# davidbau/rewriting

Measured on NVIDIA H100. Metric: StyleGAN2-256 images/sec, higher is better.
Workload: dtype bf16x3 (3-term split bf16 operands, fp32 accumulate; fp32 in/out)

## Files before the change

### rewriting_b200/csrc/conv_tc.cu

```cuda
#include <cstdlib>
#include <cstring>

#include "rw_common.cuh"
#include "rw_kernels.h"

namespace rw {

namespace {

constexpr int BM = 128;
constexpr int BK = 32;
constexpr int MMA_K = 16;
constexpr int kStages = 7;
constexpr int kNumThreads = 384;
constexpr int kTmaWarp = 8;
constexpr uint32_t kProducerRegs = 40;
constexpr uint32_t kConsumerRegs = 232;
constexpr int kCluster = 2;
constexpr int kChunkKB = 16;

template <int BN>
struct ConvSmem {
  static constexpr int kABytes = BM * BK * 2;
  static constexpr int kBBytes = BN * BK * 2;
  static constexpr int kStageBytes = 2 * kABytes + 2 * kBBytes;
  static constexpr int kTotal = kStages * kStageBytes + 512  + 256 ;
};
static_assert(ConvSmem<128>::kTotal <= 232448, "conv_tc: shared memory over the per-block limit");

struct Barriers {
  uint64_t full[kStages];
  uint64_t empty[kStages];
};

__device__ __forceinline__ void decode_tile(int tile, int nphase, int nsched, int& ph, int& mn) {
  mn = tile / nphase;
  ph = tile - mn * nphase;
  if (nphase > 1) ph = (ph + ((nsched % nphase) == 0 ? tile / nsched : mn)) % nphase;
}

template <int BN, int EPI, bool PROF>
__global__ void __launch_bounds__(kNumThreads, 1)
conv_tc_kernel(const __grid_constant__ CUtensorMap map_a_hi,
               const __grid_constant__ CUtensorMap map_a_lo,
               const __grid_constant__ CUtensorMap map_w_hi,
               const __grid_constant__ CUtensorMap map_w_lo, const ConvTcParams p) {
  extern __shared__ uint8_t smem_raw[];
  uint8_t* smem = reinterpret_cast<uint8_t*>((reinterpret_cast<uintptr_t>(smem_raw) + 511) &
                                             ~static_cast<uintptr_t>(511));
  using S = ConvSmem<BN>;
  constexpr int NR = BN / 2;
  constexpr int NJ = BN / 8;
  Barriers* bars = reinterpret_cast<Barriers*>(smem + kStages * S::kStageBytes);

  const int warp = __shfl_sync(0xffffffffu, static_cast<int>(threadIdx.x >> 5), 0);
  const int lane = threadIdx.x & 31;
  const int rank = static_cast<int>(cluster_ctarank());
  const int nsched = static_cast<int>(num_clusters_x());
  const int first_unit = static_cast<int>(cluster_id_x());

  const int m_tiles = (p.rows + BM - 1) / BM;
  const int n_tiles = p.Cout / BN;
  const int mn_units = (m_tiles + kCluster - 1) / kCluster * n_tiles;
  const int num_units = mn_units * p.nphase;
  const int kb_per_tap = p.Cin / BK;

  if (warp == kTmaWarp && lane == 0) {
    tma_prefetch_desc(&map_a_hi);
    tma_prefetch_desc(&map_a_lo);
    tma_prefetch_desc(&map_w_hi);
    tma_prefetch_desc(&map_w_lo);
    for (int s = 0; s < kStages; ++s) {
      mbar_init(&bars->full[s], 1);
      mbar_init(&bars->empty[s], 2 * kCluster);
    }
    fence_mbar_init();
  }
  cluster_sync();

  if (warp < kTmaWarp) {
    setmaxnreg_inc<kConsumerRegs>();
    const int wg = threadIdx.x >> 7;
    const int c = lane & 3;
    const int img = p.Hp * p.Wp;
    auto release = [&](int s) {
      if ((threadIdx.x & 127) == 0) {
#pragma unroll
        for (int r = 0; r < kCluster; ++r) mbar_arrive_cluster(mapa_shared(&bars->empty[s], r));
      }
    };
    auto clk = [] { return static_cast<uint32_t>(clock()); };
    uint32_t prof[6] = {0, 0, 0, 0, 0, 0};
    uint32_t tp0 = 0, tp1 = 0;
    if constexpr (PROF) prof[5] = 0u - clk();
    int stage = 0;
    uint32_t phase = 0;
    for (int unit = first_unit; unit < num_units; unit += nsched) {
      int ph, mn;
      decode_tile(unit, p.nphase, nsched, ph, mn);
      const int num_kb = p.ph_ntaps[ph] * kb_per_tap;
      const int n_tile = mn % n_tiles;
      const int n0 = n_tile * BN;
      const int m0 = ((mn / n_tiles) * kCluster + rank) * BM;

      float acc[NR], d[NR];
#pragma unroll
      for (int j = 0; j < NR; ++j) acc[j] = 0.f;
      for (int kb0 = 0; kb0 < num_kb; kb0 += kChunkKB) {
        const int kb_end = (kb0 + kChunkKB < num_kb) ? kb0 + kChunkKB : num_kb;
        int held = -1;
        for (int kb = kb0; kb < kb_end; ++kb) {
          if constexpr (PROF) tp0 = clk();
          mbar_wait(&bars->full[stage], phase);
          if constexpr (PROF) { tp1 = clk(); prof[0] += tp1 - tp0; }
          const uint32_t sa = smem_u32(smem + stage * S::kStageBytes);
          const uint64_t da_hi = make_smem_desc(sa + wg * (S::kABytes / 2), 16, 512, 2);
          const uint64_t da_lo = make_smem_desc(sa + S::kABytes + wg * (S::kABytes / 2), 16, 512, 2);
          const uint64_t db_hi = make_smem_desc(sa + 2 * S::kABytes, 16, 512, 2);
          const uint64_t db_lo = make_smem_desc(sa + 2 * S::kABytes + S::kBBytes, 16, 512, 2);
          wgmma_fence();
#pragma unroll
          for (int kk = 0; kk < BK / MMA_K; ++kk) {
            const uint64_t adv = static_cast<uint64_t>((kk * MMA_K * 2) >> 4);
            wgmma_m64nN<0, 0>(d, da_lo + adv, db_hi + adv, ((kb - kb0) | kk) != 0);
            wgmma_m64nN<0, 0>(d, da_hi + adv, db_lo + adv, 1u);
            wgmma_m64nN<0, 0>(d, da_hi + adv, db_hi + adv, 1u);
          }
          wgmma_commit();
          wgmma_wait<1>();
          if (held >= 0) release(held);
          held = stage;
          if (++stage == kStages) { stage = 0; phase ^= 1u; }
          if constexpr (PROF) prof[1] += clk() - tp1;
        }
        if constexpr (PROF) tp0 = clk();
        wgmma_wait<0>();
        release(held);
#pragma unroll
        for (int j = 0; j < NR; ++j) acc[j] += d[j];
        if constexpr (PROF) prof[2] += clk() - tp0;
      }
      if constexpr (PROF) tp0 = clk();

      uint32_t tid;
      asm volatile("mov.u32 %0, %%tid.x;\n" : "=r"(tid));
      const int row0 = m0 + ((tid >> 7) << 6) + (((tid >> 5) & 3) << 4) + ((tid & 31) >> 2);
#pragma unroll
      for (int i = 0; i < 2; ++i) {
        const int prow = row0 + 8 * i;
        const int b = prow / img;
        const int rem = prow - b * img;
        const int yy = rem / p.Wp;
        const int xx = rem - yy * p.Wp;
        const int Hv = p.ph_Hv[ph], Wv = p.ph_Wv[ph];
        const bool in_rows = prow < p.rows;
        const bool valid = in_rows && (yy < Hv) && (xx < Wv);
        const float* scl = (p.scale_bo && in_rows) ? p.scale_bo + static_cast<size_t>(b) * p.Cout : nullptr;
        float* outp = (p.out != nullptr && p.out_mode == 0 && valid)
                          ? p.out + p.ph_out_ofs[ph] + static_cast<size_t>(b) * p.out_sb +
                                static_cast<size_t>(yy) * p.out_sy + static_cast<size_t>(xx) * p.out_sx
                          : nullptr;
        if (EPI == 1 || !valid) {
          if (scl && (EPI == 1 || p.out_mode == 1)) {
#pragma unroll
            for (int j = 0; j < NJ; ++j) {
              const float2 sv = __ldg(reinterpret_cast<const float2*>(scl + n0 + 8 * j + 2 * c));
              acc[4 * j + 2 * i] *= sv.x;
              acc[4 * j + 2 * i + 1] *= sv.y;
            }
          }
          if (EPI == 1 && outp) {
#pragma unroll
            for (int j = 0; j < NJ; ++j)
#pragma unroll
              for (int e = 0; e < 2; ++e)
                outp[static_cast<size_t>(n0 + 8 * j + 2 * c + e) * p.out_sc] = acc[4 * j + 2 * i + e];
          }
        } else {
          float nz = 0.f;
          if (p.noise != nullptr)
            nz = __ldg(p.noise_w) * __ldg(p.noise + static_cast<size_t>(b) * p.noise_bstride +
                                          static_cast<size_t>(yy) * Wv + xx);
          const float act_gain = p.act_gain != 0.f ? p.act_gain : 1.4142135623730951f;
          if (scl) {
            const float* sc = scl + n0 + 2 * c;
#pragma unroll
            for (int j = 0; j < NJ; ++j)
#pragma unroll
              for (int e = 0; e < 2; ++e) acc[4 * j + 2 * i + e] *= __ldg(sc + 8 * j + e);
          }
#pragma unroll
          for (int j = 0; j < NJ; ++j)
#pragma unroll
            for (int e = 0; e < 2; ++e) acc[4 * j + 2 * i + e] += nz;
          if (p.bias) {
            const float* bi = p.bias + n0 + 2 * c;
#pragma unroll
            for (int j = 0; j < NJ; ++j)
#pragma unroll
              for (int e = 0; e < 2; ++e) acc[4 * j + 2 * i + e] += __ldg(bi + 8 * j + e);
          }
          if (p.act) {
#pragma unroll
            for (int j = 0; j < 2 * NJ; ++j) {
              float& t = acc[4 * (j >> 1) + 2 * i + (j & 1)];
              t = (t > 0.f ? t : 0.2f * t) * act_gain;
            }
          }
          if (outp) {
#pragma unroll
            for (int j = 0; j < NJ; ++j)
#pragma unroll
              for (int e = 0; e < 2; ++e)
                outp[static_cast<size_t>(n0 + 8 * j + 2 * c + e) * p.out_sc] = acc[4 * j + 2 * i + e];
          }
        }
        if (EPI == 0 && p.rgb_w != nullptr) {
          const float* rw0 = p.rgb_w + (static_cast<size_t>(valid ? b : 0) * 3) * p.Cout + n0 + 2 * c;
          const float* rw1 = rw0 + p.Cout;
          const float* rw2 = rw1 + p.Cout;
#pragma unroll
          for (int half = 0; half < BN / 64; ++half) {
            float r0 = 0.f, r1 = 0.f, r2 = 0.f;
            if (valid) {
#pragma unroll
              for (int j = 8 * half; j < 8 * half + 8; ++j)
#pragma unroll
                for (int e = 0; e < 2; ++e) {
                  const float t = acc[4 * j + 2 * i + e];
                  r0 = fmaf(__ldg(rw0 + 8 * j + e), t, r0);
                  r1 = fmaf(__ldg(rw1 + 8 * j + e), t, r1);
                  r2 = fmaf(__ldg(rw2 + 8 * j + e), t, r2);
                }
            }
#pragma unroll
            for (int s = 1; s < 4; s <<= 1) {
              r0 += __shfl_xor_sync(0xffffffffu, r0, s);
              r1 += __shfl_xor_sync(0xffffffffu, r1, s);
              r2 += __shfl_xor_sync(0xffffffffu, r2, s);
            }
            if (valid && c == 0) {
              const size_t hw = static_cast<size_t>(Hv) * Wv;
              float* rp = p.rgb_part + ((static_cast<size_t>(n_tile * (BN / 64) + half) * p.B + b) * 3) * hw +
                          static_cast<size_t>(yy) * Wv + xx;
              rp[0] = r0;
              rp[hw] = r1;
              rp[2 * hw] = r2;
            }
          }
        }
        if (p.out != nullptr && p.out_mode == 1 && in_rows) {
          float* orow = p.out + (static_cast<size_t>(ph) * p.rows + prow) * p.Cout + n0 + 2 * c;
#pragma unroll
          for (int j = 0; j < NJ; ++j)
            *reinterpret_cast<float2*>(orow + 8 * j) = make_float2(acc[4 * j + 2 * i], acc[4 * j + 2 * i + 1]);
        }
        if (EPI == 0 && p.next_hi != nullptr && in_rows) {
          const float* ns = p.next_scale + static_cast<size_t>(valid ? b : 0) * p.Cout + n0 + 2 * c;
          const size_t ofs = static_cast<size_t>(prow) * p.Cout + n0 + 2 * c;
          uint32_t* nh = reinterpret_cast<uint32_t*>(static_cast<__nv_bfloat16*>(p.next_hi) + ofs);
          uint32_t* nl = reinterpret_cast<uint32_t*>(static_cast<__nv_bfloat16*>(p.next_lo) + ofs);
#pragma unroll
          for (int j = 0; j < NJ; ++j) {
            float k0 = 0.f, k1 = 0.f;
            if (valid) {
              const float2 sv = __ldg(reinterpret_cast<const float2*>(ns + 8 * j));
              k0 = sv.x * acc[4 * j + 2 * i];
              k1 = sv.y * acc[4 * j + 2 * i + 1];
            }
            const __nv_bfloat162 hh = __floats2bfloat162_rn(k0, k1);
            const float2 hf = __bfloat1622float2(hh);
            const __nv_bfloat162 ll = __floats2bfloat162_rn(k0 - hf.x, k1 - hf.y);
            nh[4 * j] = *reinterpret_cast<const uint32_t*>(&hh);
            nl[4 * j] = *reinterpret_cast<const uint32_t*>(&ll);
          }
        }
      }
      if constexpr (PROF) { prof[3] += clk() - tp0; prof[4] += 1; }
    }
    if constexpr (PROF) {
      prof[5] += clk();
      if (lane == 0) {
        long long* dst = p.debug_prof + (static_cast<size_t>(blockIdx.x) * 8 + warp) * 8;
#pragma unroll
        for (int i = 0; i < 8; ++i) dst[i] = i < 6 ? prof[i] : 0;
      }
    }
  } else {
    setmaxnreg_dec<kProducerRegs>();
    if (warp == kTmaWarp && lane == 0) {
      constexpr uint16_t kMask = (1u << kCluster) - 1;
      constexpr int kBSlice = BN / kCluster;
      const uint32_t b_off = 2 * S::kABytes + rank * (S::kBBytes / kCluster);
      int stage = 0;
      uint32_t phase = 0;
      for (int unit = first_unit; unit < num_units; unit += nsched) {
        int ph, mn;
        decode_tile(unit, p.nphase, nsched, ph, mn);
        const int n0 = (mn % n_tiles) * BN + rank * kBSlice;
        const int m0 = ((mn / n_tiles) * kCluster + rank) * BM;
        for (int t = 0; t < p.ph_ntaps[ph]; ++t) {
          const int arow = m0 + p.ph_shift[ph][t];
          const int wcol = p.ph_kofs[ph][t];
          const int acol = p.ph_acol[ph][t];
          for (int kb = 0; kb < kb_per_tap; ++kb) {
            mbar_wait(&bars->empty[stage], phase ^ 1u);
            uint8_t* st = smem + stage * S::kStageBytes;
            mbar_expect_tx(&bars->full[stage], S::kStageBytes);
            tma_load_2d(st, &map_a_hi, &bars->full[stage], acol + kb * BK, arow);
            tma_load_2d(st + S::kABytes, &map_a_lo, &bars->full[stage], acol + kb * BK, arow);
            tma_load_2d_multicast(st + b_off, &map_w_hi, &bars->full[stage], wcol + kb * BK, n0,
                                  kMask);
            tma_load_2d_multicast(st + b_off + S::kBBytes, &map_w_lo, &bars->full[stage],
                                  wcol + kb * BK, n0, kMask);
            if (++stage == kStages) { stage = 0; phase ^= 1u; }
          }
        }
      }
    }
    __syncwarp();
  }
  cluster_sync();
}

}

template <int BN, int EPI, bool PROF>
static int conv_tc_launch_epi(const ConvTcParams& p, const void* a_hi, const void* a_lo,
                              const void* w_hi, const void* w_lo, int wk_total,
                              cudaStream_t stream) {
  CUtensorMap ma_hi, ma_lo, mw_hi, mw_lo;
  int rc;
  const uint64_t a_cols = p.a_cols > 0 ? p.a_cols : p.Cin;
  const uint64_t a_dims[2] = {a_cols, static_cast<uint64_t>(p.rows)}, a_str[1] = {a_cols * 2};
  const uint64_t w_dims[2] = {static_cast<uint64_t>(wk_total), static_cast<uint64_t>(p.Cout)};
  const uint64_t w_str[1] = {static_cast<uint64_t>(wk_total) * 2};
  const uint32_t a_box[2] = {BK, BM}, w_box[2] = {BK, BN / kCluster};
  if ((rc = make_tmap_nd_bf16(&ma_hi, a_hi, 2, a_dims, a_str, a_box, nullptr, 3))) return rc;
  if ((rc = make_tmap_nd_bf16(&ma_lo, a_lo, 2, a_dims, a_str, a_box, nullptr, 3))) return rc;
  if ((rc = make_tmap_nd_bf16(&mw_hi, w_hi, 2, w_dims, w_str, w_box, nullptr, 3))) return rc;
  if ((rc = make_tmap_nd_bf16(&mw_lo, w_lo, 2, w_dims, w_str, w_box, nullptr, 3))) return rc;

  cudaLaunchConfig_t cfg = {};
  cudaLaunchAttribute attr[1];
  attr[0].id = cudaLaunchAttributeClusterDimension;
  attr[0].val.clusterDim.x = kCluster;
  attr[0].val.clusterDim.y = 1;
  attr[0].val.clusterDim.z = 1;
  cfg.blockDim = dim3(kNumThreads);
  cfg.dynamicSmemBytes = ConvSmem<BN>::kTotal;
  cfg.stream = stream;
  cfg.attrs = attr;
  cfg.numAttrs = 1;
  static int max_clusters = 0;
  if (max_clusters == 0) {
    rc = check_cuda(cudaFuncSetAttribute(conv_tc_kernel<BN, EPI, PROF>,
                                         cudaFuncAttributeMaxDynamicSharedMemorySize, ConvSmem<BN>::kTotal),
                    "conv_tc smem attr");
    if (rc) return rc;
    cfg.gridDim = dim3(kCluster * (device_sm_count() / kCluster));
    rc = check_cuda(cudaOccupancyMaxActiveClusters(&max_clusters, conv_tc_kernel<BN, EPI, PROF>, &cfg),
                    "conv_tc cluster occupancy");
    if (rc) return rc;
    if (max_clusters < 1) {
      set_last_error("conv_tc: no cluster of %d CTAs fits on the device", kCluster);
      return RW_ERR_UNSUPPORTED;
    }
  }
  const int m_tiles = (p.rows + BM - 1) / BM;
  const int n_tiles = p.Cout / BN;
  const int num_units = (m_tiles + kCluster - 1) / kCluster * n_tiles * p.nphase;
  const int clusters = max_clusters < num_units ? max_clusters : num_units;
  cfg.gridDim = dim3(kCluster * clusters);
  rc = check_cuda(cudaLaunchKernelEx(&cfg, conv_tc_kernel<BN, EPI, PROF>, ma_hi, ma_lo, mw_hi, mw_lo, p),
                  "conv_tc launch");
  if (rc) return rc;
  return check_cuda(cudaGetLastError(), "conv_tc launch");
}

template <int BN>
static int conv_tc_launch_bn(const ConvTcParams& p, const void* a_hi, const void* a_lo,
                             const void* w_hi, const void* w_lo, int wk_total, cudaStream_t stream) {
  const bool lean = !p.noise && !p.bias && !p.act && !p.rgb_w && !p.rgb_part && !p.next_hi &&
                    p.out != nullptr && (reinterpret_cast<uintptr_t>(p.scale_bo) & 7u) == 0;
  if (p.debug_prof) return conv_tc_launch_epi<BN, 0, true>(p, a_hi, a_lo, w_hi, w_lo, wk_total, stream);
  if (lean) return conv_tc_launch_epi<BN, 1, false>(p, a_hi, a_lo, w_hi, w_lo, wk_total, stream);
  return conv_tc_launch_epi<BN, 0, false>(p, a_hi, a_lo, w_hi, w_lo, wk_total, stream);
}

int conv_tc_launch(const ConvTcParams& p, const void* a_hi, const void* a_lo, const void* w_hi,
                   const void* w_lo, int wk_total, cudaStream_t stream) {
  if (p.Cin % 64 != 0 || p.Cout % 64 != 0 || p.nphase < 1 || p.nphase > 4 || p.rows <= 0) {
    set_last_error("conv_tc: unsupported shape Cin=%d Cout=%d nphase=%d rows=%d", p.Cin, p.Cout,
                   p.nphase, p.rows);
    return RW_ERR_BAD_ARG;
  }
  for (int i = 0; i < p.nphase; ++i)
    if (p.ph_ntaps[i] < 1 || p.ph_ntaps[i] > 9) {
      set_last_error("conv_tc: phase %d has %d taps", i, p.ph_ntaps[i]);
      return RW_ERR_BAD_ARG;
    }
  const struct {
    const void* ptr;
    unsigned align;
    const char* name;
  } need[] = {
      {p.scale_bo, p.out_mode == 1 ? 8u : 4u, "scale_bo"},
      {p.out, p.out_mode == 1 ? 8u : 4u, "out"},
      {p.noise, 4u, "noise"},
      {p.noise_w, 4u, "noise_w"},
      {p.bias, 4u, "bias"},
      {p.next_scale, 8u, "next_scale"},
      {p.next_hi, 4u, "next_hi"},
      {p.next_lo, 4u, "next_lo"},
      {p.rgb_w, 4u, "rgb_w"},
      {p.rgb_part, 4u, "rgb_part"},
  };
  for (const auto& n : need)
    if (n.ptr != nullptr && (reinterpret_cast<uintptr_t>(n.ptr) & (n.align - 1)) != 0) {
      set_last_error("conv_tc: %s (%p) is not %u-byte aligned", n.name, n.ptr, n.align);
      return RW_ERR_BAD_ARG;
    }
  if (p.Cout % 128 == 0) return conv_tc_launch_bn<128>(p, a_hi, a_lo, w_hi, w_lo, wk_total, stream);
  return conv_tc_launch_bn<64>(p, a_hi, a_lo, w_hi, w_lo, wk_total, stream);
}

}
```

Measured before the change: 2046.

## Add dedicated epilogue warpgroup with shared-memory accumulator handoff

Splits the consumer into two MMA warpgroups plus a new epilogue warpgroup. MMA warps write their accumulators to a per-warpgroup shared-memory handoff buffer, signalled by acc_full/acc_empty mbarriers, so the epilogue (scaling, bf16 hi/lo split, stores) overlaps the next tile's main loop. In exchange the MMA warps get fewer registers, the block grows to 512 threads, and the BN=128 pipeline drops from 7 to 5 stages to make room for the handoff buffers, which may expose more TMA latency.

After: 2072, median of 6. 1.01x the previous value.

```diff
diff --git a/rewriting_b200/csrc/conv_tc.cu b/rewriting_b200/csrc/conv_tc.cu
--- a/rewriting_b200/csrc/conv_tc.cu
+++ b/rewriting_b200/csrc/conv_tc.cu
@@ -11,11 +11,13 @@
 constexpr int BM = 128;
 constexpr int BK = 32;
 constexpr int MMA_K = 16;
-constexpr int kStages = 7;
-constexpr int kNumThreads = 384;
-constexpr int kTmaWarp = 8;
-constexpr uint32_t kProducerRegs = 40;
-constexpr uint32_t kConsumerRegs = 232;
+constexpr int kNumThreads = 512;
+constexpr int kEpiWarp = 8;
+constexpr int kTmaWarp = 12;
+constexpr int kProfWarps = 12;
+constexpr uint32_t kMmaRegs = 184;
+constexpr uint32_t kEpiRegs = 120;
+constexpr uint32_t kProducerRegs = 24;
 constexpr int kCluster = 2;
 constexpr int kChunkKB = 16;
 
@@ -24,13 +26,20 @@
   static constexpr int kABytes = BM * BK * 2;
   static constexpr int kBBytes = BN * BK * 2;
   static constexpr int kStageBytes = 2 * kABytes + 2 * kBBytes;
-  static constexpr int kTotal = kStages * kStageBytes + 512  + 256 ;
+  static constexpr int kHandoffBytes = 64 * BN * 4;
+  static constexpr int kStages = BN == 128 ? 5 : 7;
+  static constexpr int kTotal =
+      kStages * kStageBytes + 2 * kHandoffBytes + 512  + 256 ;
 };
 static_assert(ConvSmem<128>::kTotal <= 232448, "conv_tc: shared memory over the per-block limit");
-
+static_assert(ConvSmem<64>::kTotal <= 232448, "conv_tc: shared memory over the per-block limit");
+
+template <int kStages>
 struct Barriers {
   uint64_t full[kStages];
   uint64_t empty[kStages];
+  uint64_t acc_full[2];
+  uint64_t acc_empty[2];
 };
 
 __device__ __forceinline__ void decode_tile(int tile, int nphase, int nsched, int& ph, int& mn) {
@@ -49,9 +58,12 @@
   uint8_t* smem = reinterpret_cast<uint8_t*>((reinterpret_cast<uintptr_t>(smem_raw) + 511) &
                                              ~static_cast<uintptr_t>(511));
   using S = ConvSmem<BN>;
+  constexpr int kStages = S::kStages;
   constexpr int NR = BN / 2;
   constexpr int NJ = BN / 8;
-  Barriers* bars = reinterpret_cast<Barriers*>(smem + kStages * S::kStageBytes);
+  float4* handoff = reinterpret_cast<float4*>(smem + kStages * S::kStageBytes);
+  Barriers<kStages>* bars =
+      reinterpret_cast<Barriers<kStages>*>(smem + kStages * S::kStageBytes + 2 * S::kHandoffBytes);
 
   const int warp = __shfl_sync(0xffffffffu, static_cast<int>(threadIdx.x >> 5), 0);
   const int lane = threadIdx.x & 31;
@@ -74,34 +86,33 @@
       mbar_init(&bars->full[s], 1);
       mbar_init(&bars->empty[s], 2 * kCluster);
     }
+    for (int h = 0; h < 2; ++h) {
+      mbar_init(&bars->acc_full[h], 128);
+      mbar_init(&bars->acc_empty[h], 128);
+    }
     fence_mbar_init();
   }
   cluster_sync();
 
-  if (warp < kTmaWarp) {
-    setmaxnreg_inc<kConsumerRegs>();
+  auto clk = [] { return static_cast<uint32_t>(clock()); };
+  if (warp < kEpiWarp) {
+    setmaxnreg_inc<kMmaRegs>();
     const int wg = threadIdx.x >> 7;
-    const int c = lane & 3;
-    const int img = p.Hp * p.Wp;
     auto release = [&](int s) {
       if ((threadIdx.x & 127) == 0) {
 #pragma unroll
         for (int r = 0; r < kCluster; ++r) mbar_arrive_cluster(mapa_shared(&bars->empty[s], r));
       }
     };
-    auto clk = [] { return static_cast<uint32_t>(clock()); };
-    uint32_t prof[6] = {0, 0, 0, 0, 0, 0};
+    uint32_t prof[7] = {0, 0, 0, 0, 0, 0, 0};
     uint32_t tp0 = 0, tp1 = 0;
     if constexpr (PROF) prof[5] = 0u - clk();
     int stage = 0;
-    uint32_t phase = 0;
+    uint32_t phase = 0, acc_phase = 0;
     for (int unit = first_unit; unit < num_units; unit += nsched) {
       int ph, mn;
       decode_tile(unit, p.nphase, nsched, ph, mn);
       const int num_kb = p.ph_ntaps[ph] * kb_per_tap;
-      const int n_tile = mn % n_tiles;
-      const int n0 = n_tile * BN;
-      const int m0 = ((mn / n_tiles) * kCluster + rank) * BM;
 
       float acc[NR], d[NR];
 #pragma unroll
@@ -141,12 +152,61 @@
         if constexpr (PROF) prof[2] += clk() - tp0;
       }
       if constexpr (PROF) tp0 = clk();
+      mbar_wait(&bars->acc_empty[wg], acc_phase ^ 1u);
+      if constexpr (PROF) { tp1 = clk(); prof[3] += tp1 - tp0; }
+      float4* hb = handoff + wg * (NR / 4) * 128 + (threadIdx.x & 127);
+#pragma unroll
+      for (int i = 0; i < 2; ++i)
+#pragma unroll
+        for (int jp = 0; jp < NJ / 2; ++jp)
+          hb[(i * (NJ / 2) + jp) * 128] = make_float4(acc[8 * jp + 2 * i], acc[8 * jp + 2 * i + 1],
+                                                      acc[8 * jp + 4 + 2 * i], acc[8 * jp + 5 + 2 * i]);
+      mbar_arrive(&bars->acc_full[wg]);
+      acc_phase ^= 1u;
+      if constexpr (PROF) { prof[6] += clk() - tp1; prof[4] += 1; }
+    }
+    if constexpr (PROF) {
+      prof[5] += clk();
+      if (lane == 0) {
+        long long* dst = p.debug_prof + (static_cast<size_t>(blockIdx.x) * kProfWarps + warp) * 8;
+#pragma unroll
+        for (int i = 0; i < 8; ++i) dst[i] = i < 7 ? prof[i] : 0;
+      }
+    }
+  } else if (warp < kTmaWarp) {
+    setmaxnreg_dec<kEpiRegs>();
+    const int c = lane & 3;
+    const int img = p.Hp * p.Wp;
+    uint32_t prof[6] = {0, 0, 0, 0, 0, 0};
+    uint32_t tp0 = 0, tp1 = 0;
+    if constexpr (PROF) prof[5] = 0u - clk();
+    uint32_t acc_phase = 0;
+    for (int unit = first_unit, h = 0; unit < num_units; unit += h * nsched, h ^= 1) {
+      int ph, mn;
+      decode_tile(unit, p.nphase, nsched, ph, mn);
+      const int n_tile = mn % n_tiles;
+      const int n0 = n_tile * BN;
+      const int m0 = ((mn / n_tiles) * kCluster + rank) * BM;
+      if constexpr (PROF) tp0 = clk();
+      mbar_wait(&bars->acc_full[h], acc_phase);
+      if constexpr (PROF) { tp1 = clk(); prof[0] += tp1 - tp0; }
+      const float4* hb = handoff + h * (NR / 4) * 128 + (threadIdx.x & 127);
+      float acc[NR];
 
       uint32_t tid;
       asm volatile("mov.u32 %0, %%tid.x;\n" : "=r"(tid));
-      const int row0 = m0 + ((tid >> 7) << 6) + (((tid >> 5) & 3) << 4) + ((tid & 31) >> 2);
+      const int row0 = m0 + (h << 6) + (((tid >> 5) & 3) << 4) + ((tid & 31) >> 2);
 #pragma unroll
       for (int i = 0; i < 2; ++i) {
+#pragma unroll
+        for (int jp = 0; jp < NJ / 2; ++jp) {
+          const float4 v = hb[(i * (NJ / 2) + jp) * 128];
+          acc[8 * jp + 2 * i] = v.x;
+          acc[8 * jp + 2 * i + 1] = v.y;
+          acc[8 * jp + 4 + 2 * i] = v.z;
+          acc[8 * jp + 5 + 2 * i] = v.w;
+        }
+        if (i == 1) mbar_arrive(&bars->acc_empty[h]);
         const int prow = row0 + 8 * i;
         const int b = prow / img;
         const int rem = prow - b * img;
@@ -276,12 +336,13 @@
           }
         }
       }
-      if constexpr (PROF) { prof[3] += clk() - tp0; prof[4] += 1; }
+      if constexpr (PROF) { prof[1] += clk() - tp1; prof[4] += h; }
+      acc_phase ^= h;
     }
     if constexpr (PROF) {
       prof[5] += clk();
       if (lane == 0) {
-        long long* dst = p.debug_prof + (static_cast<size_t>(blockIdx.x) * 8 + warp) * 8;
+        long long* dst = p.debug_prof + (static_cast<size_t>(blockIdx.x) * kProfWarps + warp) * 8;
 #pragma unroll
         for (int i = 0; i < 8; ++i) dst[i] = i < 6 ? prof[i] : 0;
       }
```
